# TaiseiNiman/SimpleGaussianSplat_tk71

Hardware: AMD Instinct MI355X
Metric: splat-pixel pairs blended per second (grouped cumprod fwd+bwd) (higher is better)
Workload: dtype f32; 1 GPU; cfg3: 1920x1080, 1000000 Gaussians, mean 80 splats/pixel (deep heavy-tailed lists); pairs_per_gpu=166335639, pixel_groups_per_gpu=2073600, bytes_per_pair=32, tiles_left_to_the_follow_up_kernel=0, world_size_checked=1, tiles_resolved_through_the_descriptor_tree=1258

## Files before the change

### simplegaussiansplat_tk71_amd/csrc/gcp_scan.hip

```cpp

#include <hip/hip_runtime.h>
#include <stdint.h>
#include <stdlib.h>
#include <atomic>
#include <mutex>

#include "gcp_device.hpp"
#include "grouped_cumprod_hip.h"

namespace gcp {
thread_local int t_last_hip_error = 0;
int hip_fail(hipError_t e) {
  t_last_hip_error = (int)e;
  return GCP_ERR_HIP;
}
}

namespace {
using namespace gcp;

typedef float float4_t __attribute__((ext_vector_type(4)));
typedef int int4_t __attribute__((ext_vector_type(4)));

enum : int { M_CUMPROD_FWD = 0, M_CUMSUM_FWD = 1, M_CUMPROD_BWD = 2, M_CUMSUM_REV = 3, M_CUMPROD_BWD_RECOMPUTE = 4 };

constexpr int kThreads = 256;
constexpr int kWaves = 4;
constexpr int kRows = 4;
constexpr int kTile = 1024 * kRows;
constexpr int kLbBatch = 5;
constexpr int kLbBatchBwd = 3;
constexpr int kLbChunks = ((kTile / 256 - 1) / kLbBatch) * kLbBatch + 1;
constexpr int kFixBlocks = 256;
constexpr int kFixBlocksQuiet = 32;
constexpr int kWsHeaderBytes = 256;
constexpr int kHdrEpoch = 0;
constexpr int kHdrDone = 1;
constexpr int kHdrUnresolved = 2;
constexpr int kHdrTiles = 3;
constexpr int kHdrDescResolved = 5;
constexpr int kHdrAnyUnresolved = 6;
constexpr int kHdrBarrier = 7;
constexpr unsigned kDOpen = 1u;
constexpr unsigned kDUnresolved = 2u;
constexpr unsigned kDValid = 1u << 15;
constexpr unsigned kDTree = 1u << 16;
constexpr int kLevels = 4;
constexpr int kXcdChunk = 32;
constexpr int kXcdChunkIndexed = 128;
constexpr int kDescWaitUs = 200;

static_assert(kLbChunks * 256 == kTile, "the raw look-back window is exactly the previous tile (the descriptor walk starts at the tile before it)");
static_assert((kLbChunks - 1) % kLbBatch == 0, "chunks after the first are fetched kLbBatch at a time");
static_assert((kLbChunks - 1) % kLbBatchBwd == 0, "chunks after the first are fetched kLbBatchBwd at a time in the backward");

template <int MODE>
struct Mode {
  static constexpr bool kMul = (MODE == M_CUMPROD_FWD);
  static constexpr bool kRev = (MODE == M_CUMPROD_BWD || MODE == M_CUMSUM_REV || MODE == M_CUMPROD_BWD_RECOMPUTE);
  static constexpr bool kBwd = (MODE == M_CUMPROD_BWD || MODE == M_CUMPROD_BWD_RECOMPUTE);
  static constexpr bool kRecompute = (MODE == M_CUMPROD_BWD_RECOMPUTE);
  static constexpr int kBatch = kBwd ? kLbBatchBwd : kLbBatch;
};

template <bool MUL>
struct Monoid {
  static __device__ __forceinline__ float identity() { return MUL ? 1.0f : 0.0f; }
  static __device__ __forceinline__ float op(float a, float b) { return MUL ? a * b : a + b; }
};

struct ScanArgs {
  const float* in0;
  const float* in1;
  const float* in2;
  const int* key;
  const int* ends;
  i64 n_groups;
  const float* carry;
  const int* index;
  float* out;
  i64 n;
  i64 ntiles;
  unsigned long long* desc_sets;
  i64 lvl_off[kLevels + 1];
  unsigned* hdr;
  int xcd_remap;
  long long patience;
};

template <bool MUL>
__device__ __forceinline__ float wave_seg_scan(float v, int h, int lane) {
  typedef Monoid<MUL> M;
  const float id = M::identity();
  float t;
  t = dpp_f<0x111, 0xf>(id, v); v = M::op(v, (lane - 1 >= h) ? t : id);
  t = dpp_f<0x112, 0xf>(id, v); v = M::op(v, (lane - 2 >= h) ? t : id);
  t = dpp_f<0x114, 0xf>(id, v); v = M::op(v, (lane - 4 >= h) ? t : id);
  t = dpp_f<0x118, 0xf>(id, v); v = M::op(v, (lane - 8 >= h) ? t : id);
  t = dpp_f<0x142, 0xa>(id, v); v = M::op(v, ((lane & 48) - 1 >= h) ? t : id);
  t = dpp_f<0x143, 0xc>(id, v); v = M::op(v, (31 >= h) ? t : id);
  return v;
}

__device__ __forceinline__ float wave_seg_scan_down_mul(float v, int hp, int lane) {
  float t;
  t = dpp_f<0x101, 0xf>(1.0f, v); v = v * ((lane + 1 <= hp) ? t : 1.0f);
  t = dpp_f<0x102, 0xf>(1.0f, v); v = v * ((lane + 2 <= hp) ? t : 1.0f);
  t = dpp_f<0x104, 0xf>(1.0f, v); v = v * ((lane + 4 <= hp) ? t : 1.0f);
  t = dpp_f<0x108, 0xf>(1.0f, v); v = v * ((lane + 8 <= hp) ? t : 1.0f);
#pragma unroll
  for (int q = 2; q >= 0; --q) {
    const float c = readlane_f(v, 16 * (q + 1));
    v = v * (((lane >> 4) == q && hp >= 16 * (q + 1)) ? c : 1.0f);
  }
  return v;
}

template <bool MUL>
__device__ __forceinline__ float wave_reduce(float v) {
  typedef Monoid<MUL> M;
  const float id = M::identity();
  v = M::op(v, dpp_f<0x111, 0xf>(id, v));
  v = M::op(v, dpp_f<0x112, 0xf>(id, v));
  v = M::op(v, dpp_f<0x114, 0xf>(id, v));
  v = M::op(v, dpp_f<0x118, 0xf>(id, v));
  v = M::op(v, dpp_f<0x142, 0xa>(id, v));
  v = M::op(v, dpp_f<0x143, 0xc>(id, v));
  return readlane_f(v, 63);
}

template <bool ALIGNED, bool NT = false>
__device__ __forceinline__ float4_t ld4(const float* p) {
  if (ALIGNED) {
    if (NT) return __builtin_nontemporal_load(reinterpret_cast<const float4_t*>(p));
    return *reinterpret_cast<const float4_t*>(p);
  }
  float4_t v; v.x = p[0]; v.y = p[1]; v.z = p[2]; v.w = p[3];
  return v;
}
template <bool ALIGNED, bool NT = false>
__device__ __forceinline__ int4_t ld4(const int* p) {
  if (ALIGNED) {
    if (NT) return __builtin_nontemporal_load(reinterpret_cast<const int4_t*>(p));
    return *reinterpret_cast<const int4_t*>(p);
  }
  int4_t v; v.x = p[0]; v.y = p[1]; v.z = p[2]; v.w = p[3];
  return v;
}
template <bool ALIGNED>
__device__ __forceinline__ void st4(float* p, float4_t v) {
  if (ALIGNED) {
    __builtin_nontemporal_store(v, reinterpret_cast<float4_t*>(p));
    return;
  }
  p[0] = v.x; p[1] = v.y; p[2] = v.z; p[3] = v.w;
}
__device__ __forceinline__ float4_t ld4_guard(const float* base, i64 p0, i64 n, float fill) {
  float4_t v;
  v.x = (p0 + 0 < n) ? base[p0 + 0] : fill;
  v.y = (p0 + 1 < n) ? base[p0 + 1] : fill;
  v.z = (p0 + 2 < n) ? base[p0 + 2] : fill;
  v.w = (p0 + 3 < n) ? base[p0 + 3] : fill;
  return v;
}
__device__ __forceinline__ int4_t ld4_guard(const int* base, i64 p0, i64 n, int fill) {
  int4_t v;
  v.x = (p0 + 0 < n) ? base[p0 + 0] : fill;
  v.y = (p0 + 1 < n) ? base[p0 + 1] : fill;
  v.z = (p0 + 2 < n) ? base[p0 + 2] : fill;
  v.w = (p0 + 3 < n) ? base[p0 + 3] : fill;
  return v;
}
template <bool ALIGNED, bool NT>
__device__ __forceinline__ float4_t ld4_indexed(const float* src, const int* index, i64 p, int4_t& idx) {
  idx = ld4<ALIGNED, NT>(index + p);
  float4_t v; v.x = src[idx.x]; v.y = src[idx.y]; v.z = src[idx.z]; v.w = src[idx.w];
  return v;
}
__device__ __forceinline__ float4_t ld4_indexed_guard(const float* src, const int* index, i64 p0, i64 n, float fill, int4_t& idx) {
  idx = ld4_guard(index, p0, n, 0);
  float4_t v;
  v.x = (p0 + 0 < n) ? src[idx.x] : fill;
  v.y = (p0 + 1 < n) ? src[idx.y] : fill;
  v.z = (p0 + 2 < n) ? src[idx.z] : fill;
  v.w = (p0 + 3 < n) ? src[idx.w] : fill;
  return v;
}
template <bool REV> __device__ __forceinline__ float4_t to_scan_order(float4_t v) {
  if (!REV) return v;
  float4_t r; r.x = v.w; r.y = v.z; r.z = v.y; r.w = v.x;
  return r;
}
template <bool REV> __device__ __forceinline__ int4_t to_scan_order(int4_t v) {
  if (!REV) return v;
  int4_t r; r.x = v.w; r.y = v.z; r.z = v.y; r.w = v.x;
  return r;
}

__device__ __forceinline__ i64 logical_tile(i64 b, i64 ntiles, int xcd_remap) {
  if (!xcd_remap) return b;
  const int lg = xcd_remap - 1 + 3;
  const i64 full = (ntiles >> lg) << lg;
  if (b >= full) return b;
  const i64 g = b >> lg, r = b & (((i64)1 << lg) - 1);
  return (g << lg) + ((r & 7) << (lg - 3)) + (r >> 3);
}

__device__ __forceinline__ unsigned long long pack_desc(float agg, unsigned flags, int first_head) {
  return ((unsigned long long)(flags | kDValid | ((unsigned)first_head << 2)) << 32) | __builtin_bit_cast(unsigned, agg);
}

constexpr int kEndIters = 4;
constexpr int kBitWords = 256 * kRows / 32;

__device__ __forceinline__ void wave_sync_lds() {
  __builtin_amdgcn_fence(__ATOMIC_RELEASE, "wavefront");
  __builtin_amdgcn_wave_barrier();
  __builtin_amdgcn_fence(__ATOMIC_ACQUIRE, "wavefront");
}

__device__ __forceinline__ bool group_ends(const ScanArgs& a, unsigned* bits, i64 wlo, i64 whi, int ga, int gb, int lane,
                                          i64& gend, i64& gstart) {
  if (lane < kBitWords) bits[lane] = 0u;
  wave_sync_lds();
  if (!(wlo <= whi && ga >= 0 && ga <= gb && (i64)gb < a.n_groups && (i64)gb - ga + 2 <= 64 * kEndIters)) return false;
  const int last = gb - ga + 1;
  int e[kEndIters];
#pragma unroll
  for (int it = 0; it < kEndIters; ++it) {
    const int j = it * 64 + lane;
    e[it] = 0;
    if (j <= last && ga - 1 + j >= 0) e[it] = a.ends[ga - 1 + j];
  }
  bool bad = false;
  gend = 0;
  gstart = (i64)__builtin_amdgcn_readlane(e[0], 0);
#pragma unroll
  for (int it = 0; it < kEndIters; ++it) {
    const int j = it * 64 + lane;
    const int prev = dpp_i<0x138, 0xf>(it ? __builtin_amdgcn_readlane(e[it > 0 ? it - 1 : 0], 63) : 0, e[it]);
    const i64 ej = e[it];
    if (j >= 1 && j <= last) {
      bad = bad || e[it] <= prev;
      const i64 p = ej - 1;
      if (p >= wlo && p <= whi) atomicOr(bits + ((p - wlo) >> 5), 1u << ((p - wlo) & 31));
    }
    if (j == 0) bad = bad || ej > wlo;
    if (j == 1) bad = bad || ej <= wlo;
    if (j == last - 1) bad = bad || ej > whi;
    if (j == last) bad = bad || ej <= whi;
    if ((last >> 6) == it) gend = (i64)__builtin_amdgcn_readlane(e[it], last & 63);
  }
  wave_sync_lds();
  return __ballot(bad) == 0ull;
}

template <int MODE, bool ALIGNED, bool FULL, bool CARRY, bool FIXUP = false, bool INDEXED = false, bool INPLACE = false>
__device__ __forceinline__ void scan_tile(const ScanArgs& a, const i64 lt, float* s_wv, int* s_wf,
                                          float* s_tc, int* s_fh, unsigned* s_bits, const float fix_carry = 0.0f) {
  typedef Mode<MODE> MD;
  constexpr bool REV = MD::kRev;
  constexpr bool BWD = MD::kBwd;
  constexpr bool RECOMP = MD::kRecompute;
  typedef Monoid<MD::kMul> M;
  const float id = M::identity();
  constexpr int WT = 256 * kRows;

  const int lane = threadIdx.x & 63;
  const int w = threadIdx.x >> 6;
  const i64 n = a.n;
  const i64 pt = REV ? (a.ntiles - 1 - lt) : lt;
  const i64 base = pt * (i64)kTile;
  unsigned long long* const desc = a.desc_sets + (a.hdr[kHdrEpoch] & 1u);

  const int wu = __builtin_amdgcn_readfirstlane(w);
  i64 wlo = 0, whi = -1;
  int ga = 0, gb = -1;
  if constexpr (BWD) {
    wlo = base + kTile - (i64)(wu + 1) * WT;
    whi = base + kTile - 1 - (i64)wu * WT;
    if (whi > n - 1) whi = n - 1;
  }

  const bool nt_main = w < kWaves - 1;
  float4_t v[kRows];
  int4_t kk[kRows];
  float4_t xp[BWD ? kRows : 1];
  int4_t ix[INDEXED ? kRows : 1];
  static_assert(!(INDEXED && BWD), "the backward has no indexed form");
  int4_t lb_ix;
  i64 p0[kRows];
  auto load_keys = [&](int r) {
    if (FULL) {
      if (nt_main) kk[r] = ld4<ALIGNED, true>(a.key + p0[r]);
      else kk[r] = ld4<ALIGNED>(a.key + p0[r]);
    } else {
      kk[r] = ld4_guard(a.key, p0[r], n, 0);
    }
    kk[r] = to_scan_order<REV>(kk[r]);
  };
#pragma unroll
  for (int r = 0; r < kRows; ++r) {
    const int q = w * WT + r * 256 + lane * 4;
    p0[r] = REV ? (base + kTile - 4 - q) : (base + q);
    if constexpr (!BWD) load_keys(r);
    if (FULL) {
      if (nt_main) {
        if constexpr (RECOMP) {
          v[r] = ld4<ALIGNED, true>(a.in2 + p0[r]);
        } else if constexpr (BWD) {
          v[r] = ld4<ALIGNED, true>(a.in2 + p0[r]) * ld4<ALIGNED, true>(a.in1 + p0[r]);
        } else if constexpr (INDEXED) {
          v[r] = ld4_indexed<ALIGNED, true>(a.in0, a.index, p0[r], ix[r]);
        } else {
          v[r] = ld4<ALIGNED, true>(a.in0 + p0[r]);
        }
      } else {
        if constexpr (RECOMP) {
          v[r] = ld4<ALIGNED>(a.in2 + p0[r]);
        } else if constexpr (BWD) {
          v[r] = ld4<ALIGNED>(a.in2 + p0[r]) * ld4<ALIGNED>(a.in1 + p0[r]);
        } else if constexpr (INDEXED) {
          v[r] = ld4_indexed<ALIGNED, false>(a.in0, a.index, p0[r], ix[r]);
        } else {
          v[r] = ld4<ALIGNED>(a.in0 + p0[r]);
        }
      }
      if constexpr (BWD) xp[r] = ld4<ALIGNED, true>(a.in0 + p0[r]);
    } else {
      if constexpr (RECOMP) {
        v[r] = ld4_guard(a.in2, p0[r], n, 0.0f);
        xp[r] = ld4_guard(a.in0, p0[r], n, 1.0f);
      } else if constexpr (BWD) {
        const float4_t g = ld4_guard(a.in2, p0[r], n, 0.0f);
        const float4_t c = ld4_guard(a.in1, p0[r], n, 0.0f);
        xp[r] = ld4_guard(a.in0, p0[r], n, 1.0f);
        v[r] = g * c;
      } else if constexpr (INDEXED) {
        v[r] = ld4_indexed_guard(a.in0, a.index, p0[r], n, id, ix[r]);
      } else {
        v[r] = ld4_guard(a.in0, p0[r], n, id);
      }
    }
    v[r] = to_scan_order<REV>(v[r]);
    if constexpr (BWD) xp[r] = to_scan_order<REV>(xp[r]);
  }

  if constexpr (BWD) {
    if (wlo <= whi) { ga = a.key[wlo]; gb = a.key[whi]; }
  }
  float anchor = 1.0f;
  if constexpr (RECOMP) {
    if (wlo > 0 && wlo <= whi) anchor = a.in1[wlo - 1];
  }

  const i64 pn = REV ? (base + kTile - (i64)w * WT) : (base + (i64)w * WT - 1);
  const bool nb_exists = (pn >= 0) && (pn < n);
  int nbk = 0;
  if (!BWD && nb_exists) nbk = a.key[pn];

  const bool do_lb = !FIXUP && !INPLACE && (w == 0) && (lt > 0);
  float4_t lbv = {id, id, id, id};
  float4_t lbc = {id, id, id, id};
  int4_t lbk = {0, 0, 0, 0};
  i64 lbp = 0;
  if (do_lb) {
    lbp = REV ? (base + kTile + lane * 4) : (base - (lane * 4 + 4));
    if (!REV) {
      lbk = ld4<ALIGNED>(a.key + lbp);
      if constexpr (BWD) lbv = ld4<ALIGNED>(a.in2 + lbp) * ld4<ALIGNED>(a.in1 + lbp);
      else if constexpr (INDEXED) lbv = ld4_indexed<ALIGNED, false>(a.in0, a.index, lbp, lb_ix);
      else lbv = ld4<ALIGNED>(a.in0 + lbp);
    } else if (BWD && base + kTile + 256 <= n) {
      lbv = ld4<ALIGNED>(a.in2 + lbp);
      lbc = ld4<ALIGNED>(a.in1 + lbp);
    } else {
      if constexpr (!BWD) lbk = ld4_guard(a.key, lbp, n, 0);
      if constexpr (BWD) { lbv = ld4_guard(a.in2, lbp, n, 0.0f); lbc = ld4_guard(a.in1, lbp, n, 0.0f); }
      else if constexpr (INDEXED) lbv = ld4_indexed_guard(a.in0, a.index, lbp, n, id, lb_ix);
      else lbv = ld4_guard(a.in0, lbp, n, id);
    }
  }

  bool from_ends = false;
  i64 gend = 0;
  unsigned* const wbits = s_bits + kBitWords * wu;
  i64 gstart = 0;
  int kbelow = 0;
  if constexpr (BWD) {
    from_ends = group_ends(a, wbits, wlo, whi, ga, gb, lane, gend, gstart);
    if (!from_ends) {
#pragma unroll
      for (int r = 0; r < kRows; ++r) load_keys(r);
      if (nb_exists) nbk = a.key[pn];
      if (do_lb) lbk = ld4_guard(a.key, lbp, n, 0);
      if constexpr (RECOMP) {
        if (wlo > 0 && wlo <= whi) kbelow = a.key[wlo - 1];
      }
    }
  }

  float s[kRows][4];
  float eloc[kRows];
  float rowtot[kRows];
  unsigned long long hmask[kRows];
  unsigned openbits = 0;
  unsigned lanes_open = 0;

  unsigned ebits = 0;
  if constexpr (RECOMP) {
    unsigned long long e3[kRows];
#pragma unroll
    for (int r = 0; r < kRows; ++r) {
      unsigned nib;
      if (from_ends) {
        const int off = WT - 4 - r * 256 - lane * 4;
        nib = (wbits[off >> 5] >> (off & 31)) & 0xfu;
      } else {
        const int up = (r == 0) ? nbk : __builtin_amdgcn_readlane(kk[r > 0 ? r - 1 : 0].w, 63);
        const int pk = dpp_i<0x138, 0xf>(up, kk[r].w);
        nib = (unsigned)(kk[r].w != kk[r].z) | ((unsigned)(kk[r].z != kk[r].y) << 1) | ((unsigned)(kk[r].y != kk[r].x) << 2) |
              ((unsigned)(kk[r].x != pk) << 3);
      }
      if (FULL) {
        if ((lt == 0) && (w == 0) && (r == 0) && (lane == 0)) nib |= 8u;
      } else {
        const i64 m = n - p0[r];
        nib = (m >= 4) ? (m == 4 ? (nib | 8u) : nib) : (m <= 0 ? 0u : ((nib | (1u << (m - 1))) & ((1u << m) - 1u)));
      }
      ebits |= nib << (4 * r);
      e3[r] = __ballot((nib & 8u) != 0u);
    }
    const bool low_head = (wlo == 0) || (from_ends ? (gstart == wlo) : (kbelow != ga));
    float C = anchor;
#pragma unroll
    for (int r = kRows - 1; r >= 0; --r) {
      const bool below = (r == kRows - 1) ? low_head : ((e3[r < kRows - 1 ? r + 1 : r] & 1ull) != 0ull);
      const bool F0 = (lane == 63) ? below : (((e3[r] >> 1) >> lane) & 1ull) != 0ull;
      const bool F1 = (ebits >> (4 * r)) & 1u, F2 = (ebits >> (4 * r + 1)) & 1u, F3 = (ebits >> (4 * r + 2)) & 1u;
      const float q0 = xp[r].w;
      const float q1 = F1 ? xp[r].z : q0 * xp[r].z;
      const float q2 = F2 ? xp[r].y : q1 * xp[r].y;
      const float q3 = F3 ? xp[r].x : q2 * xp[r].x;
      const bool n0 = !F0, n1 = n0 && !F1, n2 = n1 && !F2, n3 = n2 && !F3;
      const unsigned long long pm = __ballot(!n3);
      const unsigned long long from = pm >> lane;
      const int hp = from ? lane + __builtin_ctzll(from) : 64;
      const float inc = wave_seg_scan_down_mul(q3, hp, lane);
      const float ex = dpp_f<0x130, 0xf>(1.0f, inc);
      const float e = (((pm >> 1) >> lane) == 0ull) ? C * ex : ex;
      v[r].w *= n0 ? e * q0 : q0;
      v[r].z *= n1 ? e * q1 : q1;
      v[r].y *= n2 ? e * q2 : q2;
      v[r].x *= n3 ? e * q3 : q3;
      const float tot = readlane_f(inc, 0);
      C = pm ? tot : C * tot;
    }
  }

#pragma unroll
  for (int r = 0; r < kRows; ++r) {
    int lane0_prev;
    if (r == 0) lane0_prev = nbk;
    else lane0_prev = __builtin_amdgcn_readlane(kk[r - 1].w, 63);
    const int pk = dpp_i<0x138, 0xf>(lane0_prev, kk[r].w);

    bool f0, f1, f2, f3;
    if constexpr (RECOMP) {
      f0 = (ebits >> (4 * r + 3)) & 1u; f1 = (ebits >> (4 * r + 2)) & 1u; f2 = (ebits >> (4 * r + 1)) & 1u; f3 = (ebits >> (4 * r)) & 1u;
    } else if (BWD && from_ends) {
      const int off = WT - 4 - r * 256 - lane * 4;
      const unsigned nib = (wbits[off >> 5] >> (off & 31)) & 0xfu;
      f0 = (nib >> 3) & 1u; f1 = (nib >> 2) & 1u; f2 = (nib >> 1) & 1u; f3 = nib & 1u;
      if (FULL) {
        f0 = f0 || ((lt == 0) && (w == 0) && (r == 0) && (lane == 0));
      } else {
        const i64 p = p0[r];
        f0 = (p + 3 < n) && (f0 || p + 3 == n - 1);
        f1 = (p + 2 < n) && (f1 || p + 2 == n - 1);
        f2 = (p + 1 < n) && (f2 || p + 1 == n - 1);
        f3 = (p + 0 < n) && (f3 || p + 0 == n - 1);
      }
    } else if (FULL) {
      const bool first_of_array = (lt == 0) && (w == 0) && (r == 0) && (lane == 0);
      f0 = first_of_array || (kk[r].x != pk);
      f1 = kk[r].y != kk[r].x;
      f2 = kk[r].z != kk[r].y;
      f3 = kk[r].w != kk[r].z;
    } else {
      bool val[4], pex[4];
#pragma unroll
      for (int k = 0; k < 4; ++k) {
        const i64 p = REV ? (p0[r] + 3 - k) : (p0[r] + k);
        val[k] = p < n;
        pex[k] = REV ? (p + 1 < n) : (p > 0);
      }
      f0 = val[0] && (!pex[0] || kk[r].x != pk);
      f1 = val[1] && (!pex[1] || kk[r].y != kk[r].x);
      f2 = val[2] && (!pex[2] || kk[r].z != kk[r].y);
      f3 = val[3] && (!pex[3] || kk[r].w != kk[r].z);
    }
    if constexpr (CARRY) {
      if (f0) v[r].x = M::op(a.carry[kk[r].x], v[r].x);
      if (f1) v[r].y = M::op(a.carry[kk[r].y], v[r].y);
      if (f2) v[r].z = M::op(a.carry[kk[r].z], v[r].z);
      if (f3) v[r].w = M::op(a.carry[kk[r].w], v[r].w);
    }
    const float s0 = v[r].x;
    const float s1 = f1 ? v[r].y : M::op(s0, v[r].y);
    const float s2 = f2 ? v[r].z : M::op(s1, v[r].z);
    const float s3 = f3 ? v[r].w : M::op(s2, v[r].w);
    s[r][0] = s0; s[r][1] = s1; s[r][2] = s2; s[r][3] = s3;
    const bool m0 = !f0, m1 = m0 && !f1, m2 = m1 && !f2, m3 = m2 && !f3;
    openbits |= ((unsigned)m0 | ((unsigned)m1 << 1) | ((unsigned)m2 << 2) | ((unsigned)m3 << 3)) << (4 * r);

    const unsigned long long mask = __ballot(!m3);
    hmask[r] = mask;
    const unsigned long long upto = mask & (~0ull >> (63 - lane));
    const int h = upto ? (63 - __clzll(upto)) : -1;
    if ((mask & ((1ull << lane) - 1ull)) == 0ull) lanes_open |= 1u << r;

    const float inc = wave_seg_scan<MD::kMul>(s3, h, lane);
    eloc[r] = dpp_f<0x138, 0xf>(id, inc);
    rowtot[r] = readlane_f(inc, 63);
  }

  float wagg = id;
  bool whead = false;
#pragma unroll
  for (int r = 0; r < kRows; ++r) {
    wagg = hmask[r] ? rowtot[r] : M::op(wagg, rowtot[r]);
    whead = whead || (hmask[r] != 0ull);
  }
  int wfh = WT;
#pragma unroll
  for (int r = kRows - 1; r >= 0; --r) {
    if (hmask[r]) {
      const int hl = __builtin_ctzll(hmask[r]);
      const unsigned ob = (unsigned)__builtin_amdgcn_readlane((int)openbits, hl);
      wfh = r * 256 + hl * 4 + __builtin_popcount((ob >> (4 * r)) & 0xfu);
    }
  }
  if (lane == 0) { s_wv[w] = wagg; s_wf[w] = whead ? 1 : 0; s_fh[w] = wfh; }

  if (w == 0) {
    float tc = FIXUP ? fix_carry : id;
    int unresolved = 0;
    if (do_lb) {
      const int k0 = from_ends ? 0 : __builtin_amdgcn_readfirstlane(kk[0].x);
      auto process = [&](float4_t cv, int4_t ck, i64 cp, int j) -> bool {
        const float4_t lv = REV ? cv : to_scan_order<true>(cv);
        const int4_t lk = REV ? ck : to_scan_order<true>(ck);
        bool c0, c1, c2, c3;
        if (!REV) {
          c0 = lk.x == k0; c1 = lk.y == k0; c2 = lk.z == k0; c3 = lk.w == k0;
        } else if (BWD && from_ends) {
          const i64 m = (gend < n ? gend : n) - cp;
          c0 = m > 0; c1 = m > 1; c2 = m > 2; c3 = m > 3;
        } else {
          c0 = (cp + 0 < n) && lk.x == k0; c1 = (cp + 1 < n) && lk.y == k0;
          c2 = (cp + 2 < n) && lk.z == k0; c3 = (cp + 3 < n) && lk.w == k0;
        }
        float p = id;
        bool full = false;
        if (c0) { p = lv.x; if (c1) { p = M::op(p, lv.y); if (c2) { p = M::op(p, lv.z); if (c3) { p = M::op(p, lv.w); full = true; } } } }
        const unsigned long long fm = __ballot(full);
        const int L = (fm == ~0ull) ? 64 : __builtin_ctzll(~fm);
        const float contrib = (lane <= L) ? p : id;
        tc = M::op(wave_reduce<MD::kMul>(contrib), tc);
        if (L < 64) return true;
        const bool more = REV ? (base + kTile + (i64)(j + 1) * 256 < n) : (base - (i64)(j + 1) * 256 > 0);
        return !more;
      };
      if constexpr (BWD) lbv = lbv * lbc;
      bool done = process(lbv, lbk, lbp, 0);
      bool wave_headless = true;
#pragma unroll
      for (int r = 0; r < kRows; ++r) wave_headless = wave_headless && (hmask[r] == 0ull);
      for (int j = 1; !done && !wave_headless && j < kLbChunks; j += MD::kBatch) {
        float4_t cv[MD::kBatch];
        int4_t ck[MD::kBatch];
        i64 cp[MD::kBatch];
#pragma unroll
        for (int c = 0; c < MD::kBatch; ++c) {
          cp[c] = REV ? (base + kTile + (i64)(j + c) * 256 + lane * 4) : (base - ((i64)(j + c) * 256 + lane * 4 + 4));
          if (!REV) {
            ck[c] = ld4<ALIGNED>(a.key + cp[c]);
            if constexpr (BWD) cv[c] = ld4<ALIGNED>(a.in2 + cp[c]) * ld4<ALIGNED>(a.in1 + cp[c]);
            else if constexpr (INDEXED) cv[c] = ld4_indexed<ALIGNED, false>(a.in0, a.index, cp[c], lb_ix);
            else cv[c] = ld4<ALIGNED>(a.in0 + cp[c]);
          } else {
            ck[c] = int4_t{0, 0, 0, 0};
            if (!(BWD && from_ends)) ck[c] = ld4_guard(a.key, cp[c], n, 0);
            if constexpr (BWD) cv[c] = ld4_guard(a.in2, cp[c], n, 0.0f) * ld4_guard(a.in1, cp[c], n, 0.0f);
            else if constexpr (INDEXED) cv[c] = ld4_indexed_guard(a.in0, a.index, cp[c], n, id, lb_ix);
            else cv[c] = ld4_guard(a.in0, cp[c], n, id);
          }
        }
#pragma unroll
        for (int c = 0; c < MD::kBatch; ++c) {
          if (!done) done = process(cv[c], ck[c], cp[c], j + c);
        }
      }
      if (!done) unresolved = 1;
      if constexpr (CARRY) {
// ... 44 lines not shown
        float acc = id;
        int lv = 0;
        while (true) {
          unsigned long long d[kLevels];
#pragma unroll
          for (int L = 0; L < kLevels; ++L) {
            const i64 self = lt >> (6 * L);
            d[L] = 0ull;
            if (lane < (int)(self & 63)) d[L] = __hip_atomic_load(entry(L, self - 1 - lane), __ATOMIC_RELAXED, __HIP_MEMORY_SCOPE_AGENT);
          }
#pragma unroll
          for (int L = 0; L < kLevels; ++L) {
            const int digit = (int)((lt >> (6 * L)) & 63);
            const unsigned fl = (unsigned)(d[L] >> 32);
            const float val = __builtin_bit_cast(float, (unsigned)d[L]);
            const bool act = lane < digit;
            const unsigned long long am = digit ? ((1ull << digit) - 1ull) : 0ull;
            const unsigned long long vm = __ballot(act && (fl & kDValid) != 0u);
            const unsigned long long cm = __ballot(act && (fl & kDValid) != 0u && (fl & kDOpen) == 0u);
            const int lf = cm ? __builtin_ctzll(cm) : 63;
            const unsigned long long want = am & ((lf >= 63) ? ~0ull : ((2ull << lf) - 1ull));
            const bool ready = (vm & want) == want;
            if (L == pub_level && L < zl && ready) {
              if (!cur_closed) cur = M::op(wave_reduce<MD::kMul>(((want >> lane) & 1ull) ? val : id), cur);
              cur_closed = cur_closed || cm != 0ull;
              if (lane == 0)
                __hip_atomic_store(entry(L + 1, lt >> (6 * (L + 1))), pack_desc(cur, cur_closed ? 0u : kDOpen, 0), __ATOMIC_RELAXED, __HIP_MEMORY_SCOPE_AGENT);
              pub_level = L + 1;
            }
            if (!resolved && L == lv && ready) {
              acc = M::op(wave_reduce<MD::kMul>(((want >> lane) & 1ull) ? val : id), acc);
              if (cm != 0ull || (lt >> (6 * (L + 1))) == 0) { tc = acc; resolved = true; }
              else lv = L + 1;
            }
          }
          if (pub_level >= zl && resolved) break;
          if (lv >= kLevels) break;
          if (wall_clock64() - t0 > (unsigned long long)a.patience) break;
          __builtin_amdgcn_s_sleep(2);
        }
      }
      if (lane == 0 && need_carry) {
        s_tc[0] = resolved ? tc : id;
        s_wf[kWaves + 1] = resolved ? 0 : 1;
        if (!resolved) a.hdr[kHdrAnyUnresolved] = 1u;
      }
    }
    __syncthreads();
  }

  float R = s_tc[0];
  const int unresolved = s_wf[kWaves + 1];
#pragma unroll
  for (int j = 0; j < kWaves; ++j)
    if (j < w) R = s_wf[j] ? s_wv[j] : M::op(R, s_wv[j]);
  if (!FIXUP && w == kWaves - 1) {
    if (lt == 0 && lane == 0) {
      a.hdr[kHdrUnresolved] = 0;
      a.hdr[kHdrDescResolved] = 0;
      a.hdr[kHdrTiles + (a.hdr[kHdrEpoch] & 1u)] = (unsigned)a.lvl_off[kLevels];
    }
    if (a.ntiles > 1) {
      int first_head;
      float agg;
      tile_summary(first_head, agg);
      const unsigned fl = (has_head ? 0u : kDOpen) | (unresolved ? kDUnresolved : 0u) | ((need_carry && !unresolved) ? kDTree : 0u);
      if (lane == 0)
        __hip_atomic_store(entry(0, lt), pack_desc(agg, fl, first_head), __ATOMIC_RELAXED, __HIP_MEMORY_SCOPE_AGENT);
      if (has_head && !need_carry && lane >= 1 && lane <= zl)
        __hip_atomic_store(entry(lvl, lt >> (6 * lvl)), pack_desc(agg, 0u, 0), __ATOMIC_RELAXED, __HIP_MEMORY_SCOPE_AGENT);
    }
  }
  if constexpr (INPLACE) {
    if (__builtin_amdgcn_readfirstlane(unresolved)) return;
  }
#pragma unroll
  for (int r = 0; r < kRows; ++r) {
    const float e = ((lanes_open >> r) & 1u) ? M::op(R, eloc[r]) : eloc[r];
    float4_t y;
    y.x = ((openbits >> (4 * r + 0)) & 1u) ? M::op(e, s[r][0]) : s[r][0];
    y.y = ((openbits >> (4 * r + 1)) & 1u) ? M::op(e, s[r][1]) : s[r][1];
    y.z = ((openbits >> (4 * r + 2)) & 1u) ? M::op(e, s[r][2]) : s[r][2];
    y.w = ((openbits >> (4 * r + 3)) & 1u) ? M::op(e, s[r][3]) : s[r][3];
    if constexpr (BWD) {
      y.x = y.x / (xp[r].x != 0.0f ? xp[r].x : 1e-8f);
      y.y = y.y / (xp[r].y != 0.0f ? xp[r].y : 1e-8f);
      y.z = y.z / (xp[r].z != 0.0f ? xp[r].z : 1e-8f);
      y.w = y.w / (xp[r].w != 0.0f ? xp[r].w : 1e-8f);
    }
    y = to_scan_order<REV>(y);
    if constexpr (INDEXED) {
      if (FULL || p0[r] + 0 < n) a.out[ix[r].x] = y.x;
      if (FULL || p0[r] + 1 < n) a.out[ix[r].y] = y.y;
      if (FULL || p0[r] + 2 < n) a.out[ix[r].z] = y.z;
      if (FULL || p0[r] + 3 < n) a.out[ix[r].w] = y.w;
    } else if (FULL) {
      st4<ALIGNED>(a.out + p0[r], y);
    } else {
      if (p0[r] + 0 < n) a.out[p0[r] + 0] = y.x;
      if (p0[r] + 1 < n) a.out[p0[r] + 1] = y.y;
      if (p0[r] + 2 < n) a.out[p0[r] + 2] = y.z;
      if (p0[r] + 3 < n) a.out[p0[r] + 3] = y.w;
    }
    R = hmask[r] ? rowtot[r] : M::op(R, rowtot[r]);
  }

}

template <int MODE>
constexpr int waves_per_simd(bool indexed, bool inplace, bool upper) {
  if (Mode<MODE>::kBwd) return 4;
  if (Mode<MODE>::kRev || indexed || inplace) return upper ? 8 : 1;
  return 6;
}
template <int MODE>
constexpr unsigned resident_tiles_lds() {
  return Mode<MODE>::kRev ? 0u : 48u * 1024u;
}
template <int MODE, bool ALIGNED, bool CARRY, bool INDEXED = false, bool INPLACE = false>
__global__ __launch_bounds__(kThreads) __attribute__((amdgpu_waves_per_eu(waves_per_simd<MODE>(INDEXED, INPLACE, false), waves_per_simd<MODE>(INDEXED, INPLACE, true))))
void gcp_scan_main(const ScanArgs a) {
  __shared__ float s_wv[kWaves];
  __shared__ int s_wf[kWaves + 2];
  __shared__ float s_tc[1];
  __shared__ int s_fh[kWaves];
  __shared__ unsigned s_bits[Mode<MODE>::kBwd ? kWaves * kBitWords : 1];
  const i64 lt = logical_tile((i64)blockIdx.x, a.ntiles, a.xcd_remap);
  const i64 pt = Mode<MODE>::kRev ? (a.ntiles - 1 - lt) : lt;
  if ((pt + 1) * (i64)kTile <= a.n) scan_tile<MODE, ALIGNED, true, CARRY, false, INDEXED, INPLACE>(a, lt, s_wv, s_wf, s_tc, s_fh, s_bits);
  else scan_tile<MODE, ALIGNED, false, CARRY, false, INDEXED, INPLACE>(a, lt, s_wv, s_wf, s_tc, s_fh, s_bits);
}

__device__ __forceinline__ unsigned long long ld_entry(const unsigned long long* p) {
  return __hip_atomic_load(p, __ATOMIC_RELAXED, __HIP_MEMORY_SCOPE_AGENT);
}

template <bool MUL>
__device__ __forceinline__ float reduce_nearest(const unsigned long long* level, i64 idx, int count, int lane, bool& closed) {
  typedef Monoid<MUL> M;
  unsigned long long d = 0ull;
  if (lane < count) d = ld_entry(level + 2 * (idx - 1 - lane));
  const unsigned fl = (unsigned)(d >> 32);
  const float val = __builtin_bit_cast(float, (unsigned)d);
  const unsigned long long am = count ? ((count >= 64) ? ~0ull : ((1ull << count) - 1ull)) : 0ull;
  const unsigned long long cm = __ballot(lane < count && (fl & kDOpen) == 0u);
  const int lf = cm ? __builtin_ctzll(cm) : 63;
  const unsigned long long want = am & ((lf >= 63) ? ~0ull : ((2ull << lf) - 1ull));
  closed = cm != 0ull;
  return wave_reduce<MUL>(((want >> lane) & 1ull) ? val : M::identity());
}

template <bool MUL>
__device__ __forceinline__ unsigned long long rebuild_entry(const unsigned long long* desc, const i64* lvl_off, int L, i64 idx, int lane) {
  typedef Monoid<MUL> M;
  const unsigned long long* level = desc + 2 * lvl_off[L - 1];
  const i64 lastc = (idx << 6) + 63;
  const unsigned long long last = ld_entry(level + 2 * lastc);
  const float lval = __builtin_bit_cast(float, (unsigned)last);
  if ((((unsigned)(last >> 32)) & kDOpen) == 0u) return pack_desc(lval, 0u, 0);
  bool closed;
  const float part = reduce_nearest<MUL>(level, lastc, 63, lane, closed);
  return pack_desc(M::op(part, lval), closed ? 0u : kDOpen, 0);
}

template <bool MUL>
__device__ __forceinline__ float tree_carry(const unsigned long long* desc, const i64* lvl_off, i64 lt, int lane) {
  typedef Monoid<MUL> M;
  float acc = M::identity();
  for (int L = 0; L < kLevels; ++L) {
    const i64 self = lt >> (6 * L);
    bool closed;
    const float part = reduce_nearest<MUL>(desc + 2 * lvl_off[L], self, (int)(self & 63), lane, closed);
    acc = M::op(part, acc);
    if (closed || (lt >> (6 * (L + 1))) == 0) break;
  }
  return acc;
}

__device__ __forceinline__ void grid_barrier(unsigned* ctr, unsigned target) {
  __syncthreads();
  if (threadIdx.x == 0) {
    __hip_atomic_fetch_add(ctr, 1u, __ATOMIC_RELEASE, __HIP_MEMORY_SCOPE_AGENT);
    while (__hip_atomic_load(ctr, __ATOMIC_ACQUIRE, __HIP_MEMORY_SCOPE_AGENT) < target) __builtin_amdgcn_s_sleep(8);
  }
  __syncthreads();
}

constexpr int kSweep = 8;
typedef unsigned long long u64x2_t __attribute__((ext_vector_type(2)));

template <int MODE, bool CARRY, bool INDEXED = false>
__global__ __launch_bounds__(kThreads) void gcp_fallback(const ScanArgs a) {
  typedef Mode<MODE> MD;
  __shared__ float s_wv[kWaves];
  __shared__ int s_wf[kWaves + 2];
  __shared__ float s_tc[1];
  __shared__ int s_fh[kWaves];
  __shared__ unsigned s_bits[MD::kBwd ? kWaves * kBitWords : 1];
  __shared__ int s_any, s_tree, s_cnt;
  __shared__ int s_tile[64];
  __shared__ float s_carry;
  const int tid = threadIdx.x, lane = tid & 63, w = tid >> 6;
  const unsigned per = ((unsigned)a.ntiles + gridDim.x - 1u) / gridDim.x;
  const i64 r0 = (i64)blockIdx.x * per;
  const i64 r1 = (r0 + per < a.ntiles) ? (r0 + per) : a.ntiles;
  auto fetch = [&](u64x2_t (&d)[kSweep], i64 b) {
#pragma unroll
    for (int k = 0; k < kSweep; ++k) {
      const i64 t = r0 + b + k * kThreads;
      d[k] = *(const u64x2_t*)(a.desc_sets + 2 * (t < r1 ? t : 0));
    }
  };
  u64x2_t d[kSweep];
  fetch(d, tid);
  const unsigned epoch = a.hdr[kHdrEpoch];
  const unsigned tiles0 = a.hdr[kHdrTiles], tiles1 = a.hdr[kHdrTiles + 1];
  const bool any = a.hdr[kHdrAnyUnresolved] != 0u;
  const unsigned set = epoch & 1u;
  unsigned long long* const desc = a.desc_sets + set;
  unsigned long long* const other = a.desc_sets + (set ^ 1u);
  const unsigned n_other = set ? tiles0 : tiles1;
  const unsigned oper = (n_other + gridDim.x - 1u) / gridDim.x;
  const i64 z0 = (i64)blockIdx.x * oper;
  const i64 z1 = (z0 + oper < (i64)n_other) ? (z0 + oper) : (i64)n_other;

  if (tid == 0) { s_any = 0; s_tree = 0; }
  __syncthreads();
  {
    int mine = 0, tree = 0;
    auto clear = [&](i64 b) {
#pragma unroll
      for (int k = 0; k < kSweep; ++k) {
        const i64 z = z0 + b + k * kThreads;
        if (z < z1) other[2 * z] = 0ull;
      }
    };
    auto count = [&](i64 b) {
#pragma unroll
      for (int k = 0; k < kSweep; ++k) {
        const unsigned fl = (r0 + b + k * kThreads < r1) ? (unsigned)((set ? d[k].y : d[k].x) >> 32) : 0u;
        mine += (int)((fl >> 1) & 1u);
        tree += (int)((fl >> 16) & 1u);
      }
    };
    clear(tid);
    count(tid);
    for (i64 b = (i64)kSweep * kThreads; r0 + b < r1 || z0 + b < z1; b += (i64)kSweep * kThreads) {
      const bool more = r0 + b < r1;
      if (more) fetch(d, b + tid);
      clear(b + tid);
      if (more) count(b + tid);
    }
    if (mine) atomicAdd(&s_any, mine);
    if (tree) atomicAdd(&s_tree, tree);
  }
  __syncthreads();
  if (tid == 0 && s_tree) atomicAdd(a.hdr + kHdrDescResolved, (unsigned)s_tree);
  if (tid == 0 && s_any) atomicAdd(a.hdr + kHdrUnresolved, (unsigned)s_any);

  if (any) {
    unsigned phase = 0;
    for (int L = 1; L < kLevels; ++L) {
      const i64 n_complete = a.ntiles >> (6 * L);
      if (n_complete == 0) break;
      unsigned long long* const level = desc + 2 * a.lvl_off[L];
      for (i64 idx = (i64)blockIdx.x * kWaves + w; idx < n_complete; idx += (i64)gridDim.x * kWaves) {
        if ((((unsigned)(ld_entry(level + 2 * idx) >> 32)) & kDValid) != 0u) continue;
        const unsigned long long e = rebuild_entry<MD::kMul>(desc, a.lvl_off, L, idx, lane);
        if (lane == 0) __hip_atomic_store(level + 2 * idx, e, __ATOMIC_RELAXED, __HIP_MEMORY_SCOPE_AGENT);
      }
      grid_barrier(a.hdr + kHdrBarrier, ++phase * gridDim.x);
    }
    if (s_any) {
      for (i64 c0 = r0; c0 < r1; c0 += 64) {
        if (w == 0) {
          const i64 t = c0 + lane;
          const bool unres = t < r1 && ((((unsigned)(ld_entry(desc + 2 * t) >> 32)) & kDUnresolved) != 0u);
          const unsigned long long um = __ballot(unres);
          if (unres) s_tile[__builtin_popcountll(um & ((1ull << lane) - 1ull))] = lane;
          if (lane == 0) s_cnt = __builtin_popcountll(um);
        }
        __syncthreads();
        const int cnt = s_cnt;
        for (int i = 0; i < cnt; ++i) {
          const i64 lt = c0 + s_tile[i];
          if (w == 0) {
            const float c = tree_carry<MD::kMul>(desc, a.lvl_off, lt, lane);
            if (lane == 0) s_carry = c;
          }
          __syncthreads();
          const float c = s_carry;
          scan_tile<MODE, false, false, CARRY, true, INDEXED>(a, lt, s_wv, s_wf, s_tc, s_fh, s_bits, c);
          __syncthreads();
        }
        __syncthreads();
      }
    }
  }

  if (tid == 0) {
    __threadfence();
    if (atomicAdd(a.hdr + kHdrDone, 1u) == gridDim.x - 1) {
      a.hdr[kHdrDone] = 0;
      a.hdr[kHdrAnyUnresolved] = 0;
      a.hdr[kHdrBarrier] = 0;
      a.hdr[kHdrEpoch] = epoch + 1u;
    }
  }
}

__global__ void gcp_check_groups_kernel(const int* inv, const int* inv_len, i64 n, i64 G,
                                        unsigned long long* bad) {
  const i64 stride = (i64)gridDim.x * blockDim.x;
  unsigned long long local = 0;
  for (i64 i = (i64)blockIdx.x * blockDim.x + threadIdx.x; i < n; i += stride) {
    const int g = inv[i];
    if (g < 0 || g >= G) { ++local; continue; }
    if (i == 0) { if (g != 0) ++local; }
    else {
      const int gp = inv[i - 1];
      if (g != gp && g != gp + 1) ++local;
      if (g == gp + 1 && gp >= 0 && gp < G && inv_len[gp] != (int)i) ++local;
    }
    if (i == n - 1) { if (g != G - 1 || inv_len[g] != (int)n) ++local; }
  }
  if (local) atomicAdd(bad, local);
}

__global__ void gcp_check_perm_kernel(const int* index, i64 n, unsigned* seen, unsigned long long* bad) {
  const i64 stride = (i64)gridDim.x * blockDim.x;
  unsigned long long local = 0;
  for (i64 i = (i64)blockIdx.x * blockDim.x + threadIdx.x; i < n; i += stride) {
    const int v = index[i];
    if (v < 0 || (i64)v >= n) { ++local; continue; }
    const unsigned bit = 1u << (v & 31);
    if (atomicOr(seen + (v >> 5), bit) & bit) ++local;
  }
  if (local) atomicAdd(bad, local);
}

__global__ void gcp_check_ids_kernel(const int* inv, i64 n, i64 G, unsigned long long* bad) {
  const i64 stride = (i64)gridDim.x * blockDim.x;
  unsigned long long local = 0;
  for (i64 i = (i64)blockIdx.x * blockDim.x + threadIdx.x; i < n; i += stride) {
    const int g = inv[i];
    if (g < 0 || (i64)g >= G) ++local;
  }
  if (local) atomicAdd(bad, local);
}

inline void ws_levels(i64 n, i64* off ) {
  const i64 t = (n + kTile - 1) / kTile;
  off[0] = 0;
  for (int L = 0; L < kLevels; ++L) off[L + 1] = off[L] + (t > 0 ? ((t - 1) >> (6 * L)) + 1 : 1);
}

size_t ws_bytes_for(i64 n) {
  i64 off[kLevels + 1];
  ws_levels(n > 0 ? n : 0, off);
  return ((size_t)kWsHeaderBytes + (size_t)off[kLevels] * 2u * 8u + 255u) / 256u * 256u;
}

struct InternalWs {
  void* ptr = nullptr;
  size_t bytes = 0;
};
std::mutex g_ws_mutex;
InternalWs g_ws[64];

int get_internal_ws(size_t need, hipStream_t stream, void** out) {
  int dev = 0;
  GCP_HIP(hipGetDevice(&dev));
  if (dev < 0 || dev >= 64) return GCP_ERR_INVALID_ARGUMENT;
  std::lock_guard<std::mutex> lock(g_ws_mutex);
  InternalWs& w = g_ws[dev];
// ... 385 lines not shown
```

Baseline: 234.5 billion pairs/s.

## Use scalar mask-driven segmented scans and packed division in backward scan

Rewrites the segmented down-multiply scan and adds a backward-only segmented add scan. Per-lane segment-boundary comparisons are replaced by 64-bit masks built once from the head ballot and applied through inverse_ballot, so the predicate work moves to scalar registers. The backward division is expanded into a paired IEEE div_scale/rcp/fma/fixup sequence on two-element vectors, which may let the compiler use packed FMA. The group-ends loop also skips iterations past the last group. The mask arithmetic adds scalar instructions and carries some risk of segment-boundary mistakes.

```diff
diff --git a/simplegaussiansplat_tk71_amd/csrc/gcp_scan.hip b/simplegaussiansplat_tk71_amd/csrc/gcp_scan.hip
--- a/simplegaussiansplat_tk71_amd/csrc/gcp_scan.hip
+++ b/simplegaussiansplat_tk71_amd/csrc/gcp_scan.hip
@@ -102,18 +102,79 @@
   return v;
 }
 
-__device__ __forceinline__ float wave_seg_scan_down_mul(float v, int hp, int lane) {
-  float t;
-  t = dpp_f<0x101, 0xf>(1.0f, v); v = v * ((lane + 1 <= hp) ? t : 1.0f);
-  t = dpp_f<0x102, 0xf>(1.0f, v); v = v * ((lane + 2 <= hp) ? t : 1.0f);
-  t = dpp_f<0x104, 0xf>(1.0f, v); v = v * ((lane + 4 <= hp) ? t : 1.0f);
-  t = dpp_f<0x108, 0xf>(1.0f, v); v = v * ((lane + 8 <= hp) ? t : 1.0f);
+template <int K>
+__device__ __forceinline__ float seg_step_add(float v, unsigned long long z) {
+  const float t = __builtin_bit_cast(float, __builtin_amdgcn_update_dpp(0, __builtin_bit_cast(int, v), 0x110 + K, 0xf, 0xf, true));
+  return v + (__builtin_amdgcn_inverse_ballot_w64(~z) ? t : 0.0f);
+}
+__device__ __forceinline__ float wave_seg_scan_add_masks(float v, unsigned long long pm) {
+  unsigned long long z = pm;
+  v = seg_step_add<1>(v, z);
+  z |= z << 1;
+  v = seg_step_add<2>(v, z);
+  z |= z << 2;
+  v = seg_step_add<4>(v, z);
+  z |= z << 4;
+  v = seg_step_add<8>(v, z);
+  auto below_head = [](unsigned bits, unsigned all) -> unsigned { return bits ? ((1u << __builtin_ctz(bits)) - 1u) : all; };
+  const unsigned long long m15 = ((unsigned long long)below_head((unsigned)(pm >> 16) & 0xffffu, 0xffffu) << 16) |
+                                 ((unsigned long long)below_head((unsigned)(pm >> 48) & 0xffffu, 0xffffu) << 48);
+  float t = __builtin_bit_cast(float, __builtin_amdgcn_update_dpp(0, __builtin_bit_cast(int, v), 0x142, 0xf, 0xf, true));
+  v = v + (__builtin_amdgcn_inverse_ballot_w64(m15) ? t : 0.0f);
+  const unsigned long long m31 = (unsigned long long)below_head((unsigned)(pm >> 32), 0xffffffffu) << 32;
+  t = __builtin_bit_cast(float, __builtin_amdgcn_update_dpp(0, __builtin_bit_cast(int, v), 0x143, 0xf, 0xf, true));
+  v = v + (__builtin_amdgcn_inverse_ballot_w64(m31) ? t : 0.0f);
+  return v;
+}
+
+template <int K>
+__device__ __forceinline__ float seg_step_down_mul(float v, unsigned long long z) {
+  constexpr unsigned long long in_row = 0x0001000100010001ull * (0xffffu >> K);
+  const float m = v * __builtin_bit_cast(float, __builtin_amdgcn_update_dpp(0, __builtin_bit_cast(int, v), 0x100 + K, 0xf, 0xf, true));
+  return __builtin_amdgcn_inverse_ballot_w64(~z & in_row) ? m : v;
+}
+__device__ __forceinline__ float wave_seg_scan_down_mul(float v, unsigned long long pm) {
+  float m;
+  unsigned long long z = pm;
+  v = seg_step_down_mul<1>(v, z);
+  z |= z >> 1;
+  v = seg_step_down_mul<2>(v, z);
+  z |= z >> 2;
+  v = seg_step_down_mul<4>(v, z);
+  z |= z >> 4;
+  v = seg_step_down_mul<8>(v, z);
 #pragma unroll
   for (int q = 2; q >= 0; --q) {
     const float c = readlane_f(v, 16 * (q + 1));
-    v = v * (((lane >> 4) == q && hp >= 16 * (q + 1)) ? c : 1.0f);
+    const unsigned row = (unsigned)(pm >> (16 * q)) & 0xffffu;
+    const unsigned open = row ? (0xffffu & ~((2u << (31 - __builtin_clz(row))) - 1u)) : 0xffffu;
+    m = v * c;
+    v = __builtin_amdgcn_inverse_ballot_w64((unsigned long long)open << (16 * q)) ? m : v;
   }
   return v;
+}
+
+typedef float float2_t __attribute__((ext_vector_type(2)));
+__device__ __forceinline__ float2_t div2(float2_t n, float2_t d) {
+  bool s0, s1, unused;
+  float2_t ds, ns, r;
+  ds.x = __builtin_amdgcn_div_scalef(n.x, d.x, false, &unused);
+  ds.y = __builtin_amdgcn_div_scalef(n.y, d.y, false, &unused);
+  ns.x = __builtin_amdgcn_div_scalef(n.x, d.x, true, &s0);
+  ns.y = __builtin_amdgcn_div_scalef(n.y, d.y, true, &s1);
+  r.x = __builtin_amdgcn_rcpf(ds.x);
+  r.y = __builtin_amdgcn_rcpf(ds.y);
+  const float2_t one = {1.0f, 1.0f};
+  const float2_t f0 = __builtin_elementwise_fma(-ds, r, one);
+  const float2_t f1 = __builtin_elementwise_fma(f0, r, r);
+  const float2_t mul = ns * f1;
+  const float2_t f2 = __builtin_elementwise_fma(-ds, mul, ns);
+  const float2_t f3 = __builtin_elementwise_fma(f2, f1, mul);
+  const float2_t f4 = __builtin_elementwise_fma(-ds, f3, ns);
+  float2_t q;
+  q.x = __builtin_amdgcn_div_fixupf(__builtin_amdgcn_div_fmasf(f4.x, f1.x, f3.x, s0), d.x, n.x);
+  q.y = __builtin_amdgcn_div_fixupf(__builtin_amdgcn_div_fmasf(f4.y, f1.y, f3.y, s1), d.y, n.y);
+  return q;
 }
 
 template <bool MUL>
@@ -237,6 +298,7 @@
   gstart = (i64)__builtin_amdgcn_readlane(e[0], 0);
 #pragma unroll
   for (int it = 0; it < kEndIters; ++it) {
+    if (it > 0 && it * 64 > last) continue;
     const int j = it * 64 + lane;
     const int prev = dpp_i<0x138, 0xf>(it ? __builtin_amdgcn_readlane(e[it > 0 ? it - 1 : 0], 63) : 0, e[it]);
     const i64 ej = e[it];
@@ -436,7 +498,7 @@
 #pragma unroll
     for (int r = kRows - 1; r >= 0; --r) {
       const bool below = (r == kRows - 1) ? low_head : ((e3[r < kRows - 1 ? r + 1 : r] & 1ull) != 0ull);
-      const bool F0 = (lane == 63) ? below : (((e3[r] >> 1) >> lane) & 1ull) != 0ull;
+      const bool F0 = __builtin_amdgcn_inverse_ballot_w64((e3[r] >> 1) | (below ? 1ull << 63 : 0ull));
       const bool F1 = (ebits >> (4 * r)) & 1u, F2 = (ebits >> (4 * r + 1)) & 1u, F3 = (ebits >> (4 * r + 2)) & 1u;
       const float q0 = xp[r].w;
       const float q1 = F1 ? xp[r].z : q0 * xp[r].z;
@@ -444,11 +506,10 @@
       const float q3 = F3 ? xp[r].x : q2 * xp[r].x;
       const bool n0 = !F0, n1 = n0 && !F1, n2 = n1 && !F2, n3 = n2 && !F3;
       const unsigned long long pm = __ballot(!n3);
-      const unsigned long long from = pm >> lane;
-      const int hp = from ? lane + __builtin_ctzll(from) : 64;
-      const float inc = wave_seg_scan_down_mul(q3, hp, lane);
+      const float inc = wave_seg_scan_down_mul(q3, pm);
       const float ex = dpp_f<0x130, 0xf>(1.0f, inc);
-      const float e = (((pm >> 1) >> lane) == 0ull) ? C * ex : ex;
+      const unsigned long long carried = pm ? (~0ull << (63 - __builtin_clzll(pm))) : ~0ull;
+      const float e = __builtin_amdgcn_inverse_ballot_w64(carried) ? C * ex : ex;
       v[r].w *= n0 ? e * q0 : q0;
       v[r].z *= n1 ? e * q1 : q1;
       v[r].y *= n2 ? e * q2 : q2;
@@ -518,9 +579,15 @@
     hmask[r] = mask;
     const unsigned long long upto = mask & (~0ull >> (63 - lane));
     const int h = upto ? (63 - __clzll(upto)) : -1;
-    if ((mask & ((1ull << lane) - 1ull)) == 0ull) lanes_open |= 1u << r;
-
-    const float inc = wave_seg_scan<MD::kMul>(s3, h, lane);
+    if constexpr (BWD) {
+      if (__builtin_amdgcn_inverse_ballot_w64(mask ? ((2ull << __builtin_ctzll(mask)) - 1ull) : ~0ull)) lanes_open |= 1u << r;
+    } else {
+      if ((mask & ((1ull << lane) - 1ull)) == 0ull) lanes_open |= 1u << r;
+    }
+
+    float inc;
+    if constexpr (BWD) inc = wave_seg_scan_add_masks(s3, mask);
+    else inc = wave_seg_scan<MD::kMul>(s3, h, lane);
     eloc[r] = dpp_f<0x138, 0xf>(id, inc);
     rowtot[r] = readlane_f(inc, 63);
   }
@@ -732,10 +799,9 @@
     y.z = ((openbits >> (4 * r + 2)) & 1u) ? M::op(e, s[r][2]) : s[r][2];
     y.w = ((openbits >> (4 * r + 3)) & 1u) ? M::op(e, s[r][3]) : s[r][3];
     if constexpr (BWD) {
-      y.x = y.x / (xp[r].x != 0.0f ? xp[r].x : 1e-8f);
-      y.y = y.y / (xp[r].y != 0.0f ? xp[r].y : 1e-8f);
-      y.z = y.z / (xp[r].z != 0.0f ? xp[r].z : 1e-8f);
-      y.w = y.w / (xp[r].w != 0.0f ? xp[r].w : 1e-8f);
+      const float2_t lo = div2(float2_t{y.x, y.y}, float2_t{xp[r].x != 0.0f ? xp[r].x : 1e-8f, xp[r].y != 0.0f ? xp[r].y : 1e-8f});
+      const float2_t hi = div2(float2_t{y.z, y.w}, float2_t{xp[r].z != 0.0f ? xp[r].z : 1e-8f, xp[r].w != 0.0f ? xp[r].w : 1e-8f});
+      y.x = lo.x; y.y = lo.y; y.z = hi.x; y.w = hi.y;
     }
     y = to_scan_order<REV>(y);
     if constexpr (INDEXED) {
```

Measured after the change: 233.9 billion pairs/s. About the same (-0.3%).

## Transpose recompute-mode forward scan through LDS so each lane scans 16 contiguous elements

Applied to the files above, without the earlier changes.

In the backward-recompute mode, the per-row reverse segmented product scan is replaced. Each wave now writes its inputs and segment-end bits into a swizzled LDS exchange buffer, lets each lane serially scan 16 contiguous elements, does one wave-level segmented scan, then writes the results back and transposes them into row order. This replaces kRows rounds of ballots and down-scans with a single wave scan, cutting cross-lane work. In exchange it adds LDS traffic, wave barriers and 8KB of shared memory per wave, which can lower occupancy.

```diff
diff --git a/simplegaussiansplat_tk71_amd/csrc/gcp_scan.hip b/simplegaussiansplat_tk71_amd/csrc/gcp_scan.hip
--- a/simplegaussiansplat_tk71_amd/csrc/gcp_scan.hip
+++ b/simplegaussiansplat_tk71_amd/csrc/gcp_scan.hip
@@ -102,20 +102,6 @@
   return v;
 }
 
-__device__ __forceinline__ float wave_seg_scan_down_mul(float v, int hp, int lane) {
-  float t;
-  t = dpp_f<0x101, 0xf>(1.0f, v); v = v * ((lane + 1 <= hp) ? t : 1.0f);
-  t = dpp_f<0x102, 0xf>(1.0f, v); v = v * ((lane + 2 <= hp) ? t : 1.0f);
-  t = dpp_f<0x104, 0xf>(1.0f, v); v = v * ((lane + 4 <= hp) ? t : 1.0f);
-  t = dpp_f<0x108, 0xf>(1.0f, v); v = v * ((lane + 8 <= hp) ? t : 1.0f);
-#pragma unroll
-  for (int q = 2; q >= 0; --q) {
-    const float c = readlane_f(v, 16 * (q + 1));
-    v = v * (((lane >> 4) == q && hp >= 16 * (q + 1)) ? c : 1.0f);
-  }
-  return v;
-}
-
 template <bool MUL>
 __device__ __forceinline__ float wave_reduce(float v) {
   typedef Monoid<MUL> M;
@@ -219,6 +205,8 @@
   __builtin_amdgcn_fence(__ATOMIC_ACQUIRE, "wavefront");
 }
 
+__device__ __forceinline__ int lds_unit(int u) { return u ^ (((u >> 4) ^ ((u >> 2) & 2)) & 3); }
+
 __device__ __forceinline__ bool group_ends(const ScanArgs& a, unsigned* bits, i64 wlo, i64 whi, int ga, int gb, int lane,
                                           i64& gend, i64& gstart) {
   if (lane < kBitWords) bits[lane] = 0u;
@@ -257,7 +245,7 @@
 
 template <int MODE, bool ALIGNED, bool FULL, bool CARRY, bool FIXUP = false, bool INDEXED = false, bool INPLACE = false>
 __device__ __forceinline__ void scan_tile(const ScanArgs& a, const i64 lt, float* s_wv, int* s_wf,
-                                          float* s_tc, int* s_fh, unsigned* s_bits, const float fix_carry = 0.0f) {
+                                          float* s_tc, int* s_fh, unsigned* s_bits, float4_t* s_xch, const float fix_carry = 0.0f) {
   typedef Mode<MODE> MD;
   constexpr bool REV = MD::kRev;
   constexpr bool BWD = MD::kBwd;
@@ -409,7 +397,6 @@
 
   unsigned ebits = 0;
   if constexpr (RECOMP) {
-    unsigned long long e3[kRows];
 #pragma unroll
     for (int r = 0; r < kRows; ++r) {
       unsigned nib;
@@ -429,33 +416,58 @@
         nib = (m >= 4) ? (m == 4 ? (nib | 8u) : nib) : (m <= 0 ? 0u : ((nib | (1u << (m - 1))) & ((1u << m) - 1u)));
       }
       ebits |= nib << (4 * r);
-      e3[r] = __ballot((nib & 8u) != 0u);
     }
     const bool low_head = (wlo == 0) || (from_ends ? (gstart == wlo) : (kbelow != ga));
-    float C = anchor;
-#pragma unroll
-    for (int r = kRows - 1; r >= 0; --r) {
-      const bool below = (r == kRows - 1) ? low_head : ((e3[r < kRows - 1 ? r + 1 : r] & 1ull) != 0ull);
-      const bool F0 = (lane == 63) ? below : (((e3[r] >> 1) >> lane) & 1ull) != 0ull;
-      const bool F1 = (ebits >> (4 * r)) & 1u, F2 = (ebits >> (4 * r + 1)) & 1u, F3 = (ebits >> (4 * r + 2)) & 1u;
-      const float q0 = xp[r].w;
-      const float q1 = F1 ? xp[r].z : q0 * xp[r].z;
-      const float q2 = F2 ? xp[r].y : q1 * xp[r].y;
-      const float q3 = F3 ? xp[r].x : q2 * xp[r].x;
-      const bool n0 = !F0, n1 = n0 && !F1, n2 = n1 && !F2, n3 = n2 && !F3;
-      const unsigned long long pm = __ballot(!n3);
-      const unsigned long long from = pm >> lane;
-      const int hp = from ? lane + __builtin_ctzll(from) : 64;
-      const float inc = wave_seg_scan_down_mul(q3, hp, lane);
-      const float ex = dpp_f<0x130, 0xf>(1.0f, inc);
-      const float e = (((pm >> 1) >> lane) == 0ull) ? C * ex : ex;
-      v[r].w *= n0 ? e * q0 : q0;
-      v[r].z *= n1 ? e * q1 : q1;
-      v[r].y *= n2 ? e * q2 : q2;
-      v[r].x *= n3 ? e * q3 : q3;
-      const float tot = readlane_f(inc, 0);
-      C = pm ? tot : C * tot;
-    }
+    const int u0 = 255 - lane;
+    const int su0 = lds_unit(u0);
+    const int sl0 = lds_unit(4 * lane);
+    if (!from_ends) {
+      if (lane < kBitWords) wbits[lane] = 0u;
+      wave_sync_lds();
+#pragma unroll
+      for (int r = 0; r < kRows; ++r) {
+        const int u = u0 - 64 * r;
+        atomicOr(wbits + (u >> 3), ((ebits >> (4 * r)) & 0xfu) << (4 * (u & 7)));
+      }
+    }
+    float4_t* const xpar = s_xch + 512 * wu;
+    float4_t* const xy = xpar + 256;
+#pragma unroll
+    for (int r = 0; r < kRows; ++r) xpar[su0 - 64 * r] = to_scan_order<true>(xp[r]);
+    wave_sync_lds();
+    unsigned F;
+    {
+      const unsigned hi = wbits[lane >> 1];
+      unsigned lo = wbits[lane >= 2 ? (lane >> 1) - 1 : 0];
+      if (lane < 2) lo = low_head ? 0x80000000u : 0u;
+      F = (unsigned)(((((unsigned long long)hi) << 32) | lo) >> (31 + 16 * (lane & 1))) & 0xffffu;
+      if (!FULL) {
+        const i64 m = n - (wlo + 16 * lane);
+        if (m < 16) F = (m < 0) ? 0u : ((F | (1u << m)) & ((2u << m) - 1u));
+      }
+    }
+    float q[16];
+#pragma unroll
+    for (int j = 0; j < 4; ++j) {
+      const float4_t t = xpar[sl0 ^ j];
+      q[4 * j] = t.x; q[4 * j + 1] = t.y; q[4 * j + 2] = t.z; q[4 * j + 3] = t.w;
+    }
+#pragma unroll
+    for (int k = 1; k < 16; ++k) q[k] = ((F >> k) & 1u) ? q[k] : q[k - 1] * q[k];
+    const unsigned long long pm = __ballot(F != 0u);
+    const unsigned long long upto = pm & (~0ull >> (63 - lane));
+    const int h = upto ? (63 - __clzll(upto)) : -1;
+    const float inc = wave_seg_scan<true>(q[15], h, lane);
+    float e = dpp_f<0x138, 0xf>(1.0f, inc);
+    if ((pm & ((1ull << lane) - 1ull)) == 0ull) e = anchor * e;
+    const int t = F ? __builtin_ctz(F) : 16;
+#pragma unroll
+    for (int k = 0; k < 16; ++k) q[k] = (k < t) ? e * q[k] : q[k];
+#pragma unroll
+    for (int j = 0; j < 4; ++j) xy[sl0 ^ j] = float4_t{q[4 * j], q[4 * j + 1], q[4 * j + 2], q[4 * j + 3]};
+    wave_sync_lds();
+#pragma unroll
+    for (int r = 0; r < kRows; ++r) v[r] = v[r] * to_scan_order<true>(xy[su0 - 64 * r]);
   }
 
 #pragma unroll
@@ -731,6 +743,7 @@
     y.y = ((openbits >> (4 * r + 1)) & 1u) ? M::op(e, s[r][1]) : s[r][1];
     y.z = ((openbits >> (4 * r + 2)) & 1u) ? M::op(e, s[r][2]) : s[r][2];
     y.w = ((openbits >> (4 * r + 3)) & 1u) ? M::op(e, s[r][3]) : s[r][3];
+    if constexpr (RECOMP) xp[r] = to_scan_order<true>(s_xch[512 * wu + lds_unit(255 - lane) - 64 * r]);
     if constexpr (BWD) {
       y.x = y.x / (xp[r].x != 0.0f ? xp[r].x : 1e-8f);
       y.y = y.y / (xp[r].y != 0.0f ? xp[r].y : 1e-8f);
@@ -774,10 +787,11 @@
   __shared__ float s_tc[1];
   __shared__ int s_fh[kWaves];
   __shared__ unsigned s_bits[Mode<MODE>::kBwd ? kWaves * kBitWords : 1];
+  __shared__ float4_t s_xch[Mode<MODE>::kRecompute ? kWaves * 512 : 1];
   const i64 lt = logical_tile((i64)blockIdx.x, a.ntiles, a.xcd_remap);
   const i64 pt = Mode<MODE>::kRev ? (a.ntiles - 1 - lt) : lt;
-  if ((pt + 1) * (i64)kTile <= a.n) scan_tile<MODE, ALIGNED, true, CARRY, false, INDEXED, INPLACE>(a, lt, s_wv, s_wf, s_tc, s_fh, s_bits);
-  else scan_tile<MODE, ALIGNED, false, CARRY, false, INDEXED, INPLACE>(a, lt, s_wv, s_wf, s_tc, s_fh, s_bits);
+  if ((pt + 1) * (i64)kTile <= a.n) scan_tile<MODE, ALIGNED, true, CARRY, false, INDEXED, INPLACE>(a, lt, s_wv, s_wf, s_tc, s_fh, s_bits, s_xch);
+  else scan_tile<MODE, ALIGNED, false, CARRY, false, INDEXED, INPLACE>(a, lt, s_wv, s_wf, s_tc, s_fh, s_bits, s_xch);
 }
 
 __device__ __forceinline__ unsigned long long ld_entry(const unsigned long long* p) {
@@ -846,6 +860,7 @@
   __shared__ float s_tc[1];
   __shared__ int s_fh[kWaves];
   __shared__ unsigned s_bits[MD::kBwd ? kWaves * kBitWords : 1];
+  __shared__ float4_t s_xch[MD::kRecompute ? kWaves * 512 : 1];
   __shared__ int s_any, s_tree, s_cnt;
   __shared__ int s_tile[64];
   __shared__ float s_carry;
@@ -939,7 +954,7 @@
           }
           __syncthreads();
           const float c = s_carry;
-          scan_tile<MODE, false, false, CARRY, true, INDEXED>(a, lt, s_wv, s_wf, s_tc, s_fh, s_bits, c);
+          scan_tile<MODE, false, false, CARRY, true, INDEXED>(a, lt, s_wv, s_wf, s_tc, s_fh, s_bits, s_xch, c);
           __syncthreads();
         }
         __syncthreads();
```

Result: faster. 234.5 billion pairs/s before, 237.0 billion pairs/s after, median of 6 (+1.1%).
